# pomonam/LearnablePoolingMethods

Hardware: AMD Instinct MI355X
Metric: clips/sec training step, NetVladV1 K=256 300-frame 1152-d, bs=80, 1/2/4/8 GPU (higher is better)
Workload: dtype f32

## Files before the change

include/lpm_hip.h:

```cpp
#ifndef LPM_HIP_H
#define LPM_HIP_H

#include <stddef.h>
#include <stdint.h>

#ifdef __cplusplus
extern "C" {
#endif

#define LPM_VERSION 100

typedef void* lpm_stream_t;

enum {
    LPM_OK = 0,
    LPM_ERR_BADARG = -1,
    LPM_ERR_UNSUPPORTED_SHAPE = -2,
    LPM_ERR_WORKSPACE = -3,
    LPM_ERR_LAUNCH = -4
};

enum {
    LPM_VLAD_SOFTMAX = 1,
    LPM_VLAD_RESIDUAL = 2,
// ... 352 lines not shown
                          const float* corr_b, float* dk, int64_t ldd, const float* moments, lpm_stream_t stream);
int lpm_mha_bwd_x3_bn_image_fmt(const float* q, const float* k, const float* v, int64_t ld, const float* o, const float* dout, int64_t ldo,
                                const float* lse, int B, int L, int h, int d, float scale, const float* key_scale, const float* key_shift,
                                float* dk_plain, const float* corr_a, const float* corr_b, float* dz_partial, void* dqkv_img,
                                const LpmOperandFormat* g_fmt, lpm_stream_t stream);
int lpm_mha_bn_dk_correct_image(const float* q, const float* k, int64_t ld, int B, int L, int h, int d, float scale, const float* corr_a,
                                const float* corr_b, const float* dk_plain, const float* moments, void* dqkv_img,
                                const LpmOperandFormat* g_fmt, lpm_stream_t stream);
int lpm_mha_logit_stats_moments(const float* q, const float* k, int64_t ld, int B, int L, int h, int d, float* partial, float* moments,
                                lpm_stream_t stream);
int lpm_mha_bwd_x3_image(const float* q, const float* k, const float* v, int64_t ld, const void* o, int o_is_image,
                         const float* dout, int64_t ldo, const float* lse, int B, int L, int h, int d, float scale, void* dqkv3,
                         lpm_stream_t stream);
int lpm_mha_fwd_x3_image(const float* q, const float* k, const float* v, int64_t ld, int B, int L, int h, int d, float scale,
                         void* o3, float* lse, lpm_stream_t stream);
size_t lpm_mha_logit_stats_workspace_bytes(int B, int L, int h);
int lpm_mha_logit_stats(const float* q, const float* k, int64_t ld, int B, int L, int h, int d, float* partial,
                        lpm_stream_t stream);
int lpm_bn_small_fwd(const float* x, int M, int C, const float* gamma, const float* beta, float eps, float decay, int act,
                     const float* mul, float* y, float* mean, float* rstd, float* moving_mean, float* moving_var, lpm_stream_t stream);
int lpm_bn_small_bwd(const float* dy, const float* x, int M, int C, const float* gamma, const float* beta, const float* mean,
                     const float* rstd, int act, const float* mul, float* dx, float* dgamma, float* dbeta, float* dmul,
                     lpm_stream_t stream);
int lpm_mha_bn_corrections(const float* partial, int nblk, int L, const float* mean, const float* var, const float* kscale, float eps,
                           int64_t n, float* dgamma, float* dbeta, float* corr_a, float* corr_b, lpm_stream_t stream);

int lpm_moe_ce_nblk(int B, int V);
int lpm_moe_ce_fwd(const float* gate_act, const float* expert_act, const float* labels, int B, int V, int num_mixtures, float eps,
                   float* predictions, float* loss, float* loss_partial, lpm_stream_t stream);
int lpm_moe_ce_bwd(const float* gate_act, const float* expert_act, const float* labels, const float* dloss,
                   const float* dpredictions, int B, int V, int num_mixtures, float eps, float* dgate_act, float* dexpert_act,
                   lpm_stream_t stream);

#define LPM_ARENA_ALIGN 4096
size_t lpm_clip_adam_scratch_bytes(int64_t total, int ntensors);
int lpm_multi_tensor_clip_adam(float* param, const float* grad, float* m, float* v, const int64_t* offsets,
                               int ntensors, int64_t total, float clip_norm, float lr, float beta1, float beta2,
                               float eps, int64_t step, float* scratch, lpm_stream_t stream);
int lpm_multi_tensor_clip_adam_l2(float* param, const float* grad, float* m, float* v, const int64_t* offsets, const float* l2coef,
                                  int ntensors, int64_t total, float clip_norm, float lr, float beta1, float beta2, float eps,
                                  int64_t step, float* scratch, lpm_stream_t stream);

size_t lpm_factored_clip_adam_scratch_bytes(int N1, int N2);
int lpm_factored_clip_adam(const void* xt, const void* dyt, int R, int N1, int N2, float* param, float* m, float* v,
                           float clip_norm, float lr, float beta1, float beta2, float eps, int64_t step, float* scratch,
                           size_t scratch_bytes, lpm_stream_t stream);
int lpm_factored_clip_adam_q(const void* xt, const void* dyt, const float* x, int64_t ldx, const void* gdt, int R, int N1, int N2,
                             float* param, float* m, float* v, float clip_norm, float lr, float beta1, float beta2, float eps,
                             int64_t step, float* scratch, size_t scratch_bytes, lpm_stream_t stream);
int lpm_factored_clip_adam_copy(const void* xt, const void* dyt, const float* x, int64_t ldx, const void* gdt, int R, int N1, int N2,
                                float* param, float* m, float* v, void* param_bf16, float clip_norm, float lr, float beta1, float beta2,
                                float eps, int64_t step, float* scratch, size_t scratch_bytes, lpm_stream_t stream);
int lpm_factored_fold_supported(int R, int N1, int N2);
int lpm_factored_clip_adam_copy_dx(const void* xt, const void* dyt, const float* x, int64_t ldx, const void* gdt, int R, int N1, int N2,
                                   float* param, float* m, float* v, void* param_bf16, const void* dy_bf16, float* dx, int64_t ld_dx,
                                   float clip_norm, float lr, float beta1, float beta2, float eps, int64_t step, float* scratch,
                                   size_t scratch_bytes, lpm_stream_t stream);

int lpm_dropout_keep_mask(void* mask, int64_t n, float keep_prob, uint64_t seed, lpm_stream_t stream);

int lpm_topk_rows(const float* p, int B, int V, int k, int32_t* index, float* value, lpm_stream_t stream);

int lpm_eval_rows(const float* p, const unsigned char* labels, int B, int V, int k, unsigned char* hit1, int32_t* num_labels,
                  int32_t* hits_at_n, double* loss_row, int32_t* top_index, float* top_value, unsigned char* top_label, lpm_stream_t stream);

#ifdef __cplusplus
// ... 4 lines not shown
```

learnablepoolingmethods_amd/_capi.py:

```python
from __future__ import annotations

import ctypes as C
import os
from typing import Optional

import torch

_HERE = os.path.dirname(os.path.abspath(__file__))
LIB_PATH = os.path.join(_HERE, "_lib", "liblpm_hip.so")

LPM_VLAD_SOFTMAX = 1
LPM_VLAD_RESIDUAL = 2
LPM_VLAD_OUT_KMAJOR = 4
LPM_VLAD_NRM_RAW = 8
LPM_VLAD_OUT_BF16 = 16
LPM_VLAD_TILES_BF16 = 32
LPM_VLAD_NRM_BF16 = 64
LPM_VLAD_RAW_KMAJOR = 128
LPM_VLAD_DEBUG_FALLBACK = 256
LPM_VLAD_WIDE_ALL = 512
LPM_VLAD_WIDE_NONE = 1024

_f = C.c_void_p
_i = C.c_int
# ... 113 lines not shown
    "lpm_bn_rows_fwd": (_i, [_f, _i, _i, _f, _f, _fl, _fl, _i, _f, _f, _f, _f, _f, _f, _s, _f]),
    "lpm_bn_bwd_workspace_bytes": (_s, [_i, _i]),
    "lpm_bn_bwd": (_i, [_f, _f, _f, _f, _f, _fl, _i, _i, _f, _f, _f, _f, _s, _f]),
    "lpm_bn_bwd_x16": (_i, [_f, _f, _f, _f, _f, _fl, _i, _i, _f, _f, _f, _f, _s, _f]),
    "lpm_split_rows": (_i, [_f, _l, _l, _i, _f, _i, _i, _f, _f]),
    "lpm_split_weight": (_i, [_f, _i, _i, _f, _f, _f]),
    "lpm_split_rows_relu_bwd_workspace_bytes": (_s, [_l, _i]),
    "lpm_bias_act_fwd": (_i, [_f, _f, _i, _l, _i, _f]),
    "lpm_bias_act_bwd_workspace_bytes": (_s, [_l, _i]),
    "lpm_bias_act_bwd": (_i, [_f, _f, _i, _l, _i, _f, _f, _f, _s, _f]),
    "lpm_split_rows_relu_bwd": (_i, [_f, _l, _i, _f, _f, _f, _f, _s, _f]),
    "lpm_layer_norm_workspace_bytes": (_s, [_i, _i]),
    "lpm_layer_norm_fwd": (_i, [_f, _f, _f, _f, _i, _i, _i, _fl, _f, _f, _f, _f, _s, _f]),
    "lpm_layer_norm_bwd": (_i, [_f, _f, _f, _f, _i, _i, _i, _f, _f, _f, _f, _s, _f]),
    "lpm_layer_norm_act_fwd": (_i, [_f, _f, _i, _f, _f, _f, _i, _i, _i, _fl, _f, _l, _f, _f, _f, _s, _f]),
    "lpm_layer_norm_pair_fwd": (_i, [_f, _f, _i, _f, _f, _f, _f, _f, _i, _i, _i, _fl, _f, _l, _f, _f, _f, _f, _f, _s, _f]),
    "lpm_layer_norm_act_bwd": (_i, [_f, _l, _f, _f, _f, _f, _f, _i, _i, _i, _i, _f, _f, _f, _f, _f, _f, _f, _f, _s, _f]),
    "lpm_layer_norm_act_mask_image_fwd": (_i, [_f, _f, _i, _f, _fl, _f, _f, _f, _i, _i, _i, _fl, _f, _l, _f, _f, _f, _f, _s, _f]),
    "lpm_layer_norm_act_mask_bwd": (_i, [_f, _l, _f, _f, _f, _f, _f, _i, _f, _fl, _i, _i, _i, _f, _f, _f, _f, _f, _f, _f, _f, _s, _f]),
    "lpm_layer_norm_act_mask_bwd_fmt": (_i, [_f, _l, _f, _f, _f, _f, _f, _i, _f, _fl, _i, _i, _i, _f, _f, _f, _f, _f, _f, _f, _f, _s, _f, _f]),
    "lpm_mha_fwd": (_i, [_f, _f, _f, _l, _i, _i, _i, _i, _fl, _f, _f, _f, _l, _f, _f]),
    "lpm_mha_fwd_x3": (_i, [_f, _f, _f, _l, _i, _i, _i, _i, _fl, _f, _f, _f, _l, _f, _f]),
    "lpm_mha_bwd": (_i, [_f, _f, _f, _l, _f, _f, _l, _f, _i, _i, _i, _i, _fl, _f, _f, _f, _f, _f, _l, _f, _f, _f, _f]),
    "lpm_mha_bn_dk_correct": (_i, [_f, _f, _l, _i, _i, _i, _i, _fl, _f, _f, _f, _l, _f, _f]),
    "lpm_mha_logit_stats_moments": (_i, [_f, _f, _l, _i, _i, _i, _i, _f, _f, _f]),
    "lpm_mha_bwd_x3": (_i, [_f, _f, _f, _l, _f, _f, _l, _f, _i, _i, _i, _i, _fl, _f, _f, _f, _f, _f, _l, _f, _f, _f, _f]),
    "lpm_mha_bwd_x3_image": (_i, [_f, _f, _f, _l, _f, _i, _f, _l, _f, _i, _i, _i, _i, _fl, _f, _f]),
    "lpm_mha_fwd_x3_image": (_i, [_f, _f, _f, _l, _i, _i, _i, _i, _fl, _f, _f, _f]),
    "lpm_mha_logit_stats_workspace_bytes": (_s, [_i, _i, _i]),
    "lpm_mha_logit_stats": (_i, [_f, _f, _l, _i, _i, _i, _i, _f, _f]),
    "lpm_moe_ce_nblk": (_i, [_i, _i]),
    "lpm_moe_ce_fwd": (_i, [_f, _f, _f, _i, _i, _i, _fl, _f, _f, _f, _f]),
    "lpm_moe_ce_bwd": (_i, [_f, _f, _f, _f, _f, _i, _i, _i, _fl, _f, _f, _f]),
    "lpm_clip_adam_scratch_bytes": (_s, [_l, _i]),
    "lpm_factored_clip_adam_scratch_bytes": (_s, [_i, _i]),
    "lpm_factored_clip_adam_q": (_i, [_f, _f, _f, _l, _f, _i, _i, _i, _f, _f, _f, _fl, _fl, _fl, _fl, _fl, _l, _f, _s, _f]),
    "lpm_factored_clip_adam_copy": (_i, [_f, _f, _f, _l, _f, _i, _i, _i, _f, _f, _f, _f, _fl, _fl, _fl, _fl, _fl, _l, _f, _s, _f]),
    "lpm_factored_clip_adam_copy_dx": (_i, [_f, _f, _f, _l, _f, _i, _i, _i, _f, _f, _f, _f, _f, _f, _l, _fl, _fl, _fl, _fl, _fl, _l, _f, _s, _f]),
    "lpm_factored_fold_supported": (_i, [_i, _i, _i]),
    "lpm_factored_clip_adam": (_i, [_f, _f, _i, _i, _i, _f, _f, _f, _fl, _fl, _fl, _fl, _fl, _l, _f, _s, _f]),
    "lpm_multi_tensor_clip_adam": (_i, [_f, _f, _f, _f, _f, _i, _l, _fl, _fl, _fl, _fl, _fl, _l, _f, _f]),
    "lpm_dropout_keep_mask": (_i, [_f, _l, _fl, C.c_uint64, _f]),
    "lpm_topk_rows": (_i, [_f, _i, _i, _i, _f, _f, _f]),
    "lpm_eval_rows": (_i, [_f, _f, _i, _i, _i, _f, _f, _f, _f, _f, _f, _f, _f]),
    "lpm_multi_tensor_clip_adam_l2": (_i, [_f, _f, _f, _f, _f, _f, _i, _l, _fl, _fl, _fl, _fl, _fl, _l, _f, _f]),
    "lpm_weight_pack": (_i, [_f, _i, _f]),
    "lpm_sum_splits": (_i, [_f, _i, _i, _i, _f, _f, _f, _i, _f]),
    "lpm_split_rows_fmt": (_i, [_f, _l, _l, _i, _f, _i, _i, _f, _f, _f, _f]),
    "lpm_split_rows_relu_bwd_fmt": (_i, [_f, _l, _i, _fl, _f, _i, _f, _f, _f, _s, _f, _f]),
    "lpm_split_weight_fmt": (_i, [_f, _i, _i, _f, _f, _i, _f]),
    "lpm_split_weight_tiles_fmt": (_i, [_f, _i, _i, _i, _f, _i, _f]),
    "lpm_split_rows_tiles_fmt": (_i, [_f, _l, _i, _i, _i, _f, _f, _f]),
    "lpm_image_row_tiles_fmt": (_i, [_f, _i, _i, _i, _f, _i, _f]),
    "lpm_dense_tiles_act_image_fwd_fmt": (_i, [_f, _i, _f, _f, _i, _i, _i, _fl, _f, _f, _f]),
    "lpm_dense_tiles_relu_bwd_image_fmt": (_i, [_f, _i, _f, _f, _i, _i, _i, _i, _fl, _f, _f, _f, _s, _f, _f]),
    "lpm_layer_norm_act_image_fwd_fmt": (_i, [_f, _f, _i, _f, _f, _f, _f, _i, _i, _i, _fl, _f, _l, _f, _f, _f, _f, _s, _f, _f]),
    "lpm_layer_norm_act_mask_image_fwd_fmt": (_i, [_f, _f, _i, _f, _fl, _f, _f, _f, _i, _i, _i, _fl, _f, _l, _f, _f, _f, _f, _s, _f, _f]),
    "lpm_layer_norm_act_bwd_fmt": (_i, [_f, _l, _f, _f, _f, _f, _f, _i, _i, _i, _i, _f, _f, _f, _f, _f, _f, _f, _f, _s, _f, _f]),
    "lpm_mha_fwd_x3_image_fmt": (_i, [_f, _f, _f, _l, _i, _i, _i, _i, _fl, _f, _f, _f, _f]),
    "lpm_mha_bwd_x3_image_fmt": (_i, [_f, _f, _f, _l, _f, _f, _f, _l, _f, _i, _i, _i, _i, _fl, _f, _f, _f]),
    "lpm_sum_splits_scaled": (_i, [_f, _i, _i, _i, _i, _fl, _f, _f, _f, _i, _f]),
    "lpm_mha_bwd_x3_bn_image_fmt": (_i, [_f, _f, _f, _l, _f, _f, _l, _f, _i, _i, _i, _i, _fl, _f, _f, _f, _f, _f, _f, _f, _f, _f]),
    "lpm_mha_bn_dk_correct_image": (_i, [_f, _f, _l, _i, _i, _i, _i, _fl, _f, _f, _f, _f, _f, _f, _f]),
    "lpm_bn_rows_act_image_fwd_fmt": (_i, [_f, _f, _i, _i, _i, _f, _f, _fl, _fl, _i, _f, _f, _f, _f, _f, _f, _s, _f, _f]),
    "lpm_bn_act_bwd_image_fmt": (_i, [_f, _f, _f, _i, _f, _f, _f, _fl, _i, _i, _f, _f, _f, _f, _f, _s, _f, _f]),
}
# ... 70 lines not shown
```

learnablepoolingmethods_amd/csrc/moe_head.hip:

```cpp
#include "lpm_common.h"

namespace lpm {

constexpr int MOE_MAX_MIX = 8;

__device__ __forceinline__ void moe_mix(const float* __restrict__ ga, const float* __restrict__ ea, int m, float* g, float* e, float* ne,
                                        float& p, float& q) {
    float mx = ga[0];
    for (int i = 1; i <= m; ++i) mx = fmaxf(mx, ga[i]);
    float s = 0.f;
    for (int i = 0; i <= m; ++i) {
        g[i] = __expf(ga[i] - mx);
        s += g[i];
    }
    const float inv = 1.f / s;
    p = 0.f;
    for (int i = 0; i <= m; ++i) g[i] *= inv;
    q = g[m];
    for (int i = 0; i < m; ++i) {
        const float a = ea[i], t = __expf(-fabsf(a)), r = 1.f / (1.f + t);
        const float big = r, small = t * r;
        e[i] = a >= 0.f ? big : small;
        ne[i] = a >= 0.f ? small : big;
        p = fmaf(g[i], e[i], p);
// ... 26 lines not shown

__global__ __launch_bounds__(256) void moe_ce_loss_reduce_kernel(const float* __restrict__ partial, int nblk, float inv_batch,
                                                                 float* __restrict__ loss) {
    __shared__ double sh[256];
    double s = 0.0;
    for (int i = threadIdx.x; i < nblk; i += 256) s += (double)partial[i];
    sh[threadIdx.x] = s;
    __syncthreads();
    for (int o = 128; o > 0; o >>= 1) {
        if (threadIdx.x < o) sh[threadIdx.x] += sh[threadIdx.x + o];
        __syncthreads();
    }
    if (threadIdx.x == 0) loss[0] = (float)(sh[0] * (double)inv_batch);
}

__global__ __launch_bounds__(256) void moe_ce_bwd_kernel(const float* __restrict__ gate_act, const float* __restrict__ expert_act,
                                                         const float* __restrict__ labels, const float* __restrict__ dloss,
                                                         const float* __restrict__ dpred, int64_t n, int m, float eps,
                                                         float inv_batch, float* __restrict__ dgate, float* __restrict__ dexpert) {
    const int64_t i = (int64_t)blockIdx.x * 256 + threadIdx.x;
    if (i >= n) return;
    float g[MOE_MAX_MIX + 1], e[MOE_MAX_MIX], ne[MOE_MAX_MIX], p, q;
    moe_mix(gate_act + i * (m + 1), expert_act + i * m, m, g, e, ne, p, q);
    float dp = dpred ? dpred[i] : 0.f;
    if (labels && dloss) {
        const float y = labels[i];
        dp += dloss[0] * inv_batch * -(y / (p + eps) - (1.f - y) / (q + eps));
    }
    for (int j = 0; j < m; ++j) {
        dexpert[i * m + j] = dp * g[j] * e[j] * ne[j];
        dgate[i * (m + 1) + j] = dp * g[j] * (q - ne[j]);
    }
    dgate[i * (m + 1) + m] = dp * g[m] * (0.f - p);
}

}

extern "C" int lpm_moe_ce_nblk(int B, int V) { return (int)(((int64_t)B * V + 255) / 256); }

extern "C" int lpm_moe_ce_fwd(const float* gate_act, const float* expert_act, const float* labels, int B, int V, int num_mixtures,
                              float eps, float* predictions, float* loss, float* loss_partial, lpm_stream_t stream) {
    using namespace lpm;
    LPM_REQUIRE(gate_act && expert_act && predictions, LPM_ERR_BADARG, "lpm_moe_ce_fwd: null pointer");
    LPM_REQUIRE((labels == nullptr) == (loss == nullptr) && (loss == nullptr) == (loss_partial == nullptr), LPM_ERR_BADARG,
                "lpm_moe_ce_fwd: labels, loss and loss_partial go together");
    LPM_REQUIRE(B > 0 && V > 0 && num_mixtures >= 1 && num_mixtures <= MOE_MAX_MIX, LPM_ERR_UNSUPPORTED_SHAPE,
                "lpm_moe_ce_fwd: need 1 <= num_mixtures <= %d (got %d)", MOE_MAX_MIX, num_mixtures);
    const int64_t n = (int64_t)B * V;
    const int nblk = lpm_moe_ce_nblk(B, V);
    hipStream_t s = (hipStream_t)stream;
    hipLaunchKernelGGL(moe_ce_fwd_kernel, dim3(nblk), dim3(256), 0, s, gate_act, expert_act, labels, n, num_mixtures, eps, predictions,
                       loss_partial);
    if (loss) hipLaunchKernelGGL(moe_ce_loss_reduce_kernel, dim3(1), dim3(256), 0, s, loss_partial, nblk, 1.f / (float)B, loss);
    return check_launch("lpm_moe_ce_fwd");
}

extern "C" int lpm_moe_ce_bwd(const float* gate_act, const float* expert_act, const float* labels, const float* dloss,
                              const float* dpredictions, int B, int V, int num_mixtures, float eps, float* dgate_act,
                              float* dexpert_act, lpm_stream_t stream) {
    using namespace lpm;
    LPM_REQUIRE(gate_act && expert_act && dgate_act && dexpert_act, LPM_ERR_BADARG, "lpm_moe_ce_bwd: null pointer");
    LPM_REQUIRE((labels == nullptr) == (dloss == nullptr), LPM_ERR_BADARG, "lpm_moe_ce_bwd: labels and dloss go together");
    LPM_REQUIRE(B > 0 && V > 0 && num_mixtures >= 1 && num_mixtures <= MOE_MAX_MIX, LPM_ERR_UNSUPPORTED_SHAPE,
                "lpm_moe_ce_bwd: need 1 <= num_mixtures <= %d (got %d)", MOE_MAX_MIX, num_mixtures);
    const int64_t n = (int64_t)B * V;
    hipLaunchKernelGGL(moe_ce_bwd_kernel, dim3(lpm_moe_ce_nblk(B, V)), dim3(256), 0, (hipStream_t)stream, gate_act, expert_act, labels, dloss,
                       dpredictions, n, num_mixtures, eps, 1.f / (float)B, dgate_act, dexpert_act);
    return check_launch("lpm_moe_ce_bwd");
}
```

learnablepoolingmethods_amd/ops.py:

```python
from __future__ import annotations

import ctypes as C
import os
import weakref
from typing import NamedTuple, Optional

import torch

from . import _capi
from ._capi import LPM_VLAD_NRM_RAW, LPM_VLAD_OUT_KMAJOR, LPM_VLAD_RESIDUAL, LPM_VLAD_SOFTMAX, LpmError, ptr, stream_ptr

BN_EPS = 1e-3
BN_DECAY = 0.999

VLAD_PRECISION = os.environ.get("LPM_VLAD_PRECISION", "bf16x3")
VLAD_TILES3 = os.environ.get("LPM_VLAD_TILES3", "1") != "0"
VLAD_FUSED = os.environ.get("LPM_VLAD_FUSED", "0") == "1"
PROJ_STREAM = os.environ.get("LPM_PROJ_STREAM", "1") != "0"
PROJ_DX_STREAM_MIN_N = int(os.environ.get("LPM_PROJ_DX_STREAM_MIN_N", "512"))
BN_ACT_FUSED = os.environ.get("LPM_BN_ACT_FUSED", "1") != "0"
BIAS_ACT_FUSED = os.environ.get("LPM_BIAS_ACT_FUSED", "1") != "0"
FACTORED_NORM_QUADFORM = os.environ.get("LPM_FACTORED_NORM_QUADFORM", "1") != "0"
VLAD_SOFTMAX_FUSED = os.environ.get("LPM_VLAD_SOFTMAX_FUSED", "0") == "1"
FRAME_ROW_TILES = os.environ.get("LPM_FRAME_ROW_TILES", "0") == "1"
VLAD_FUSED_DEBUG_FALLBACK = False

VLAD_KMAJOR_SCALED = os.environ.get("LPM_VLAD_KMAJOR_SCALED", "0") == "1"
VLAD_CLIP = os.environ.get("LPM_VLAD_CLIP", "1") != "0"
VLAD_CLIP16 = os.environ.get("LPM_VLAD_CLIP16", "1") != "0"
FFN_TILES = os.environ.get("LPM_FFN_TILES", "1") != "0"
DIRECT_WGRAD = True
FFN_MOD_FUSED = os.environ.get("LPM_FFN_MOD_FUSED", "1") != "0"
ASSIGN_PRECISION = os.environ.get("LPM_ASSIGN_PRECISION", "bf16x3")

MHA_PRECISION = os.environ.get("LPM_MHA_PRECISION", "bf16x3")
MHA_BN_PRECISION = os.environ.get("LPM_MHA_BN_PRECISION", "mixed")
MHA_BN_MIXED = os.environ.get("LPM_MHA_BN_MIXED", "auto,bf16x3,bf16x3")
MHA_BN_X3_MIN_KEYS = int(os.environ.get("LPM_MHA_BN_X3_MIN_KEYS", "128"))

_XT_CACHE = {}
MHA_BN_MOMENTS = os.environ.get("LPM_MHA_BN_MOMENTS", "1") != "0"
MHA_BN_ONEPASS = os.environ.get("LPM_MHA_BN_ONEPASS", "1") != "0"
LN_IMAGE = os.environ.get("LPM_LN_IMAGE", "1") != "0"
SPLIT_VECTOR = True
V2_SPLIT_COLUMNS = True
DEBUG_TAP = None

KERNEL_TIMELINE = None


class _timed:
    def __init__(self, name, dims):
        self.name, self.dims = name, dims

    def __enter__(self):
        if KERNEL_TIMELINE is not None:
            self.t0 = torch.cuda.Event(enable_timing=True)
            self.t1 = torch.cuda.Event(enable_timing=True)
            self.t0.record()
        return self

    def __exit__(self, *exc):
        if KERNEL_TIMELINE is not None:
            self.t1.record()
            KERNEL_TIMELINE.append((self.name, self.dims, self.t0, self.t1))
        return False


def _f32(t: torch.Tensor, what: str) -> torch.Tensor:
    if t.dtype != torch.float32:
        raise LpmError(f"{what}: expected float32, got {t.dtype}")
    return t


# ... 2888 lines not shown
        if labels is not None:
            labels = labels.to(device=gate_act.device, dtype=torch.float32).contiguous()
            loss = _empty((), gate_act)
            part = _empty((lib._lpm_moe_ce_nblk(B, V),), gate_act)
        lib.check(lib._lpm_moe_ce_fwd(ptr(gate_act), ptr(expert_act), ptr(labels), B, V, num_mixtures, eps, ptr(pred), ptr(loss),
                                      ptr(part), stream_ptr()), "lpm_moe_ce_fwd")
        ctx.dims = (B, V, num_mixtures, eps)
        ctx.save_for_backward(gate_act, expert_act, labels)
        ctx.set_materialize_grads(False)
        if labels is None:
            ctx.mark_non_differentiable()
            return pred, None
        return pred, loss

    @staticmethod
    def backward(ctx, dpred, dloss):
        lib = _capi.load()
        B, V, m, eps = ctx.dims
        gate_act, expert_act, labels = ctx.saved_tensors
        dgate, dexpert = torch.empty_like(gate_act), torch.empty_like(expert_act)
        if dloss is None and labels is not None:
            dloss = torch.zeros((), dtype=torch.float32, device=gate_act.device)
        dloss = dloss.contiguous() if dloss is not None else None
        dpred = dpred.contiguous() if dpred is not None else None
        lib.check(lib._lpm_moe_ce_bwd(ptr(gate_act), ptr(expert_act), ptr(labels), ptr(dloss), ptr(dpred), B, V, m, eps, ptr(dgate),
                                      ptr(dexpert), stream_ptr()), "lpm_moe_ce_bwd")
        return dgate, dexpert, None, None, None


def moe_cross_entropy(gate_act, expert_act, labels, num_mixtures, eps=10e-6):
    return _MoeCrossEntropy.apply(gate_act, expert_act, labels, int(num_mixtures), float(eps))


class ComputeCopy:

    def __init__(self, W, also=()):
        self.buf = torch.empty(W.shape, dtype=torch.bfloat16, device=W.device)
        self.also = tuple(also)
        self.version = None
        self.stale = True
        self.refreshes = 0

    def invalidate(self):
        self.stale = True

    def _versions(self, W):
        return (W._version,) + tuple(t._version for t in self.also)

    def tensor(self, W):
        v = self._versions(W)
        if self.stale or self.version != v:
            self.buf.copy_(W.detach())
            self.version, self.stale = v, False
            self.refreshes += 1
        return self.buf

    def current(self, W):
        return None if (self.stale or self.version != self._versions(W)) else self.buf


PROJ_W16 = os.environ.get("LPM_PROJ_W16", "1") != "0"


class FactoredGradient:

    def __init__(self, on_put=None, strict=False):
# ... 149 lines not shown
```

learnablepoolingmethods_amd/video_level_models.py:

```python
from __future__ import annotations

import math

import torch

from . import FLAGS, models
from . import variables as vs


def _linear(x, W, b=None):
    if x.is_cuda and x.dtype == torch.float32 and W.dtype == torch.float32 and x.dim() == 2:
        from . import ops
        return ops.linear_direct(x, W, b)
    return torch.addmm(b, x, W) if b is not None else x.matmul(W)


class MoeModel(models.BaseModel):

    def create_model(self, model_input, vocab_size, is_training=True, num_mixtures=None, l2_penalty=1e-8,
                     labels=None, fused_cross_entropy=False, **unused_params):
        num_mixtures = num_mixtures or FLAGS.moe_num_mixtures
        low_rank_gating = FLAGS.moe_low_rank_gating
        l2_penalty = FLAGS.moe_l2
        gating_probabilities = FLAGS.moe_prob_gating
        gating_input = FLAGS.moe_prob_gating_input
        H = model_input.shape[1]
        dev = model_input.device
        store = vs.default_store()
        if low_rank_gating == -1:
            with vs.variable_scope("gates"):
                wg = vs.get_variable("weights", [H, vocab_size * (num_mixtures + 1)], vs.glorot_uniform_initializer(), device=dev)
            store.add_l2_regularizer(wg, l2_penalty)
            gate_activations = _linear(model_input, wg)
        else:
            with vs.variable_scope("gates1"):
                wg1 = vs.get_variable("weights", [H, low_rank_gating], vs.glorot_uniform_initializer(), device=dev)
            with vs.variable_scope("gates2"):
                wg2 = vs.get_variable("weights", [low_rank_gating, vocab_size * (num_mixtures + 1)], vs.glorot_uniform_initializer(), device=dev)
            store.add_l2_regularizer(wg1, l2_penalty)
            store.add_l2_regularizer(wg2, l2_penalty)
            gate_activations = model_input.matmul(wg1).matmul(wg2)
        with vs.variable_scope("experts"):
            we = vs.get_variable("weights", [H, vocab_size * num_mixtures], vs.glorot_uniform_initializer(), device=dev)
            be = vs.get_variable("biases", [vocab_size * num_mixtures], vs.zeros_initializer(), device=dev)
        store.add_l2_regularizer(we, l2_penalty)
        expert_activations = _linear(model_input, we, be)
        fuse_loss = fused_cross_entropy and not gating_probabilities
        if model_input.is_cuda and num_mixtures <= 8 and (labels is None or fused_cross_entropy):
            from . import ops
            probabilities, loss = ops.moe_cross_entropy(gate_activations, expert_activations,
                                                        labels if fuse_loss else None, num_mixtures)
            if not gating_probabilities:
                return {"predictions": probabilities, "loss": loss} if loss is not None else {"predictions": probabilities}
        else:
            gating_distribution = torch.softmax(gate_activations.reshape(-1, num_mixtures + 1), dim=-1)
            expert_distribution = torch.sigmoid(expert_activations.reshape(-1, num_mixtures))
            probabilities = (gating_distribution[:, :num_mixtures] * expert_distribution).sum(dim=1)
            probabilities = probabilities.reshape(-1, vocab_size)
        if gating_probabilities:
            from . import layers
            rows = vocab_size if gating_input == "prob" else H
            gating_weights = vs.get_variable("gating_prob_weights", [rows, vocab_size],
                                             vs.random_normal_initializer(1 / math.sqrt(vocab_size)), device=dev)
            gates = (probabilities if gating_input == "prob" else model_input).matmul(gating_weights)
            if FLAGS.gating_remove_diag:
                if rows != vocab_size:
                    raise ValueError("gating_remove_diag with moe_prob_gating_input != 'prob': the diagonal of a "
                                     f"[{rows}, {vocab_size}] matrix does not broadcast against the probabilities (as in the reference)")
                gates = gates - torch.diagonal(gating_weights) * probabilities
            gates = layers.batch_norm(gates, is_training, "gating_prob_bn")
            probabilities = probabilities * torch.sigmoid(gates)
        return {"predictions": probabilities}
```

Baseline: 12530.

## Fuse MoE head linear layers with mixture and cross-entropy into one kernel

Adds fused forward and backward HIP kernels that compute the gate and expert linear projections with MFMA, the mixture-of-experts probabilities, and the cross-entropy loss in one pass per column block. The backward also produces weight, bias and input gradients, with input gradients written to per-block slabs and then reduced. This removes separate GEMM launches and the round trips of activations through memory. The cost is extra slab memory and reduction work for dx, plus custom GEMM code that may be slower than a library GEMM for larger shapes. It is only used for full-rank gating with batch size up to 128.

```diff
diff --git a/include/lpm_hip.h b/include/lpm_hip.h
--- a/include/lpm_hip.h
+++ b/include/lpm_hip.h
@@ -408,6 +408,15 @@
                    const float* dpredictions, int B, int V, int num_mixtures, float eps, float* dgate_act, float* dexpert_act,
                    lpm_stream_t stream);
 
+int lpm_moe_head_nblk(int V, int num_mixtures);
+int lpm_moe_head_fwd(const float* x, const float* gate_w, const float* expert_w, const float* expert_b, const void* labels,
+                     int labels_u8, int B, int H, int V, int num_mixtures, float eps, float* gate_act, float* expert_act,
+                     float* predictions, float* loss, float* loss_partial, lpm_stream_t stream);
+int lpm_moe_head_bwd(const float* x, const float* gate_w, const float* expert_w, const float* gate_act, const float* expert_act,
+                     const void* labels, int labels_u8, const float* dloss, const float* dpredictions, int B, int H, int V,
+                     int num_mixtures, float eps, float* dgate_w, float* dexpert_w, float* dexpert_b, float* dx, float* dx_slabs,
+                     lpm_stream_t stream);
+
 #define LPM_ARENA_ALIGN 4096
 size_t lpm_clip_adam_scratch_bytes(int64_t total, int ntensors);
 int lpm_multi_tensor_clip_adam(float* param, const float* grad, float* m, float* v, const int64_t* offsets,
diff --git a/learnablepoolingmethods_amd/_capi.py b/learnablepoolingmethods_amd/_capi.py
--- a/learnablepoolingmethods_amd/_capi.py
+++ b/learnablepoolingmethods_amd/_capi.py
@@ -169,6 +169,9 @@
     "lpm_moe_ce_nblk": (_i, [_i, _i]),
     "lpm_moe_ce_fwd": (_i, [_f, _f, _f, _i, _i, _i, _fl, _f, _f, _f, _f]),
     "lpm_moe_ce_bwd": (_i, [_f, _f, _f, _f, _f, _i, _i, _i, _fl, _f, _f, _f]),
+    "lpm_moe_head_nblk": (_i, [_i, _i]),
+    "lpm_moe_head_fwd": (_i, [_f, _f, _f, _f, _f, _i, _i, _i, _i, _i, _fl, _f, _f, _f, _f, _f, _f]),
+    "lpm_moe_head_bwd": (_i, [_f, _f, _f, _f, _f, _f, _i, _f, _f, _i, _i, _i, _i, _fl, _f, _f, _f, _f, _f, _f]),
     "lpm_clip_adam_scratch_bytes": (_s, [_l, _i]),
     "lpm_factored_clip_adam_scratch_bytes": (_s, [_i, _i]),
     "lpm_factored_clip_adam_q": (_i, [_f, _f, _f, _l, _f, _i, _i, _i, _f, _f, _f, _fl, _fl, _fl, _fl, _fl, _l, _f, _s, _f]),
diff --git a/learnablepoolingmethods_amd/csrc/moe_head.hip b/learnablepoolingmethods_amd/csrc/moe_head.hip
--- a/learnablepoolingmethods_amd/csrc/moe_head.hip
+++ b/learnablepoolingmethods_amd/csrc/moe_head.hip
@@ -82,6 +82,396 @@
         dgate[i * (m + 1) + j] = dp * g[j] * (q - ne[j]);
     }
     dgate[i * (m + 1) + m] = dp * g[m] * (0.f - p);
+}
+
+
+constexpr int MH_NT = 5;
+constexpr int MH_COLS = 16 * MH_NT;
+constexpr int MH_LDT = MH_COLS + 1;
+
+struct HeadCols {
+    int ng, nl;
+    int g0, e0;
+    int gN, eN;
+};
+__device__ __forceinline__ HeadCols head_cols(int blk, int cb, int m, int V) {
+    HeadCols hc;
+    hc.ng = cb * (m + 1);
+    hc.nl = cb * (2 * m + 1);
+    hc.g0 = blk * hc.ng;
+    hc.e0 = blk * cb * m;
+    hc.gN = V * (m + 1);
+    hc.eN = V * m;
+    return hc;
+}
+__device__ __forceinline__ bool head_col(const HeadCols& hc, int c, bool& expert, int& col) {
+    expert = c >= hc.ng;
+    col = expert ? hc.e0 + (c - hc.ng) : hc.g0 + c;
+    return c < hc.nl && col < (expert ? hc.eN : hc.gN);
+}
+__device__ __forceinline__ float head_label(const void* labels, int u8, int64_t i) {
+    return u8 ? (float)((const uint8_t*)labels)[i] : ((const float*)labels)[i];
+}
+
+template <int RT>
+__global__ __launch_bounds__(256) void moe_head_fwd_kernel(const float* __restrict__ x, const float* __restrict__ Wg,
+                                                           const float* __restrict__ We, const float* __restrict__ be,
+                                                           const void* __restrict__ labels, int labels_u8, int B, int H, int V, int m,
+                                                           int cb, float eps, float* __restrict__ gate_act,
+                                                           float* __restrict__ expert_act, float* __restrict__ pred,
+                                                           float* __restrict__ loss_partial) {
+    __shared__ __attribute__((aligned(16))) float T[RT * 16 * MH_LDT];
+    const int blk = xcd_remap(blockIdx.x, gridDim.x);
+    const int lane = threadIdx.x & 63, wave = threadIdx.x >> 6, li = lane & 15, g = lane >> 4;
+    const HeadCols hc = head_cols(blk, cb, m, V);
+
+    const float* wp[MH_NT];
+    int ld[MH_NT];
+#pragma unroll
+    for (int t = 0; t < MH_NT; ++t) {
+        bool ex;
+        int col;
+        const bool ok = head_col(hc, t * 16 + li, ex, col);
+        wp[t] = ok ? (ex ? We : Wg) + col : Wg;
+        ld[t] = (ok && ex) ? hc.eN : hc.gN;
+    }
+    constexpr int NIT = (RT * 16 * 26 + 255) / 256;
+    __shared__ float bias_s[MH_COLS];
+    __shared__ float ys[NIT * 256];
+    if (threadIdx.x < MH_COLS) {
+        bool ex;
+        int col;
+        const bool ok = head_col(hc, threadIdx.x, ex, col);
+        bias_s[threadIdx.x] = (ok && ex) ? be[col] : 0.f;
+    }
+    if (labels) {
+        float yv[NIT];
+        int64_t yi[NIT];
+#pragma unroll
+        for (int it = 0; it < NIT; ++it) {
+            const int i = min((int)threadIdx.x + it * 256, B * cb - 1), r = i / cb;
+            yi[it] = (int64_t)r * V + min(blk * cb + (i - r * cb), V - 1);
+        }
+        if (labels_u8) {
+#pragma unroll
+            for (int it = 0; it < NIT; ++it) yv[it] = (float)((const uint8_t*)labels)[yi[it]];
+        } else {
+#pragma unroll
+            for (int it = 0; it < NIT; ++it) yv[it] = ((const float*)labels)[yi[it]];
+        }
+#pragma unroll
+        for (int it = 0; it < NIT; ++it) ys[threadIdx.x + it * 256] = yv[it];
+    }
+
+    f32x4 acc[RT][MH_NT];
+#pragma unroll
+    for (int rt = 0; rt < RT; ++rt)
+#pragma unroll
+        for (int t = 0; t < MH_NT; ++t) acc[rt][t] = f32x4{0.f, 0.f, 0.f, 0.f};
+
+    const int nch = H >> 4, ch0 = wave * nch / 4, ch1 = (wave + 1) * nch / 4;
+    auto load = [&](int ch, float (&w)[4][MH_NT], f32x4 (&xv)[RT]) {
+        const int k = ch * 16 + 4 * g;
+#pragma unroll
+        for (int s = 0; s < 4; ++s)
+#pragma unroll
+            for (int t = 0; t < MH_NT; ++t) w[s][t] = wp[t][(int64_t)(k + s) * ld[t]];
+#pragma unroll
+        for (int rt = 0; rt < RT; ++rt) xv[rt] = *(const f32x4*)(x + (int64_t)min(rt * 16 + li, B - 1) * H + k);
+    };
+    float w0[4][MH_NT], w1[4][MH_NT], w2[4][MH_NT];
+    f32x4 x0[RT], x1[RT], x2[RT];
+    auto step = [&](int next, float (&wc)[4][MH_NT], f32x4 (&xc)[RT], float (&wn)[4][MH_NT], f32x4 (&xn)[RT]) {
+        load(min(next, ch1 - 1), wn, xn);
+        __builtin_amdgcn_sched_barrier(0);
+#pragma unroll
+        for (int s = 0; s < 4; ++s)
+#pragma unroll
+            for (int rt = 0; rt < RT; ++rt)
+#pragma unroll
+                for (int t = 0; t < MH_NT; ++t) acc[rt][t] = mfma16(xc[rt][s], wc[s][t], acc[rt][t]);
+        __builtin_amdgcn_sched_barrier(0);
+    };
+    if (ch0 < ch1) {
+        load(ch0, w0, x0);
+        load(min(ch0 + 1, ch1 - 1), w1, x1);
+        for (int ch = ch0; ch < ch1; ch += 3) {
+            step(ch + 2, w0, x0, w2, x2);
+            if (ch + 1 >= ch1) break;
+            step(ch + 3, w1, x1, w0, x0);
+            if (ch + 2 >= ch1) break;
+            step(ch + 4, w2, x2, w1, x1);
+        }
+    }
+
+    f32x4* stage = (f32x4*)T;
+    for (int src = 3; src >= 1; --src) {
+        if (wave == src) {
+#pragma unroll
+            for (int rt = 0; rt < RT; ++rt)
+#pragma unroll
+                for (int t = 0; t < MH_NT; ++t) stage[(rt * MH_NT + t) * 64 + lane] = acc[rt][t];
+        }
+        __syncthreads();
+        if (wave == src - 1) {
+#pragma unroll
+            for (int rt = 0; rt < RT; ++rt)
+#pragma unroll
+                for (int t = 0; t < MH_NT; ++t) acc[rt][t] += stage[(rt * MH_NT + t) * 64 + lane];
+        }
+    }
+    __syncthreads();
+    if (wave == 0) {
+#pragma unroll
+        for (int rt = 0; rt < RT; ++rt)
+#pragma unroll
+            for (int t = 0; t < MH_NT; ++t)
+#pragma unroll
+                for (int j = 0; j < 4; ++j) T[(rt * 16 + 4 * g + j) * MH_LDT + t * 16 + li] = acc[rt][t][j];
+    }
+    __syncthreads();
+
+    for (int i = threadIdx.x; i < B * MH_COLS; i += 256) {
+        const int r = i / MH_COLS, c = i - r * MH_COLS;
+        bool ex;
+        int col;
+        if (!head_col(hc, c, ex, col)) continue;
+        const float v = T[r * MH_LDT + c] + bias_s[c];
+        if (ex) {
+            T[r * MH_LDT + c] = v;
+            if (expert_act) expert_act[(int64_t)r * hc.eN + col] = v;
+        } else if (gate_act) {
+            gate_act[(int64_t)r * hc.gN + col] = v;
+        }
+    }
+    __syncthreads();
+    float l = 0.f;
+    for (int i = threadIdx.x; i < B * cb; i += 256) {
+        const int r = i / cb, cl = i - r * cb, cls = blk * cb + cl;
+        if (cls >= V) continue;
+        float gg[MOE_MAX_MIX + 1], e[MOE_MAX_MIX], ne[MOE_MAX_MIX], p, q;
+        moe_mix(T + r * MH_LDT + cl * (m + 1), T + r * MH_LDT + hc.ng + cl * m, m, gg, e, ne, p, q);
+        pred[(int64_t)r * V + cls] = p;
+        if (labels) {
+            const float y = ys[i];
+            l += -(y * __logf(p + eps) + (1.f - y) * __logf(q + eps));
+        }
+    }
+    if (loss_partial) {
+        l = wave_sum(l);
+        __shared__ float w[4];
+        if (lane == 0) w[wave] = l;
+        __syncthreads();
+        if (threadIdx.x == 0) loss_partial[blk] = (w[0] + w[1]) + (w[2] + w[3]);
+    }
+}
+
+template <int RT>
+__global__ __launch_bounds__(256) void moe_head_bwd_kernel(const float* __restrict__ x, const float* __restrict__ Wg,
+                                                           const float* __restrict__ We, const float* __restrict__ gate_act,
+                                                           const float* __restrict__ expert_act, const void* __restrict__ labels,
+                                                           int labels_u8, const float* __restrict__ dloss,
+                                                           const float* __restrict__ dpred, int B, int H, int V, int m, int cb, float eps,
+                                                           float* __restrict__ dWg, float* __restrict__ dWe, float* __restrict__ dbe,
+                                                           float* __restrict__ dx_slabs) {
+    __shared__ __attribute__((aligned(16))) float T[RT * 16 * MH_LDT];
+    const int blk = xcd_remap(blockIdx.x, gridDim.x);
+    const int lane = threadIdx.x & 63, wave = threadIdx.x >> 6, li = lane & 15, g = lane >> 4;
+    const HeadCols hc = head_cols(blk, cb, m, V);
+
+    constexpr int NCP = RT * 16 * MH_COLS / 256, NIT = (RT * 16 * 26 + 255) / 256;
+    const int nitem = B * cb;
+    float yv[NIT], dpv[NIT];
+    {
+        float v[NCP];
+#pragma unroll
+        for (int it = 0; it < NCP; ++it) {
+            const int i = threadIdx.x + it * 256, r = i / MH_COLS, c = i - r * MH_COLS;
+            bool ex;
+            int col;
+            const bool ok = head_col(hc, c, ex, col) && r < B;
+            const float* src = !ok ? gate_act : ex ? expert_act + (int64_t)r * hc.eN + col : gate_act + (int64_t)r * hc.gN + col;
+            v[it] = *src;
+        }
+        int64_t yi[NIT];
+#pragma unroll
+        for (int it = 0; it < NIT; ++it) {
+            const int i = min((int)threadIdx.x + it * 256, nitem - 1), r = i / cb;
+            yi[it] = (int64_t)r * V + min(blk * cb + (i - r * cb), V - 1);
+            yv[it] = 0.f;
+            dpv[it] = 0.f;
+        }
+        if (labels && dloss) {
+            if (labels_u8) {
+#pragma unroll
+                for (int it = 0; it < NIT; ++it) yv[it] = (float)((const uint8_t*)labels)[yi[it]];
+            } else {
+#pragma unroll
+                for (int it = 0; it < NIT; ++it) yv[it] = ((const float*)labels)[yi[it]];
+            }
+        }
+        if (dpred) {
+#pragma unroll
+            for (int it = 0; it < NIT; ++it) dpv[it] = dpred[yi[it]];
+        }
+#pragma unroll
+        for (int it = 0; it < NCP; ++it) {
+            const int i = threadIdx.x + it * 256, r = i / MH_COLS, c = i - r * MH_COLS;
+            bool ex;
+            int col;
+            const bool ok = head_col(hc, c, ex, col) && r < B;
+            T[r * MH_LDT + c] = ok ? v[it] : 0.f;
+        }
+    }
+    __syncthreads();
+    const float inv_batch = 1.f / (float)B, dl = (labels && dloss) ? dloss[0] * inv_batch : 0.f;
+#pragma unroll
+    for (int it = 0; it < NIT; ++it) {
+        const int i = threadIdx.x + it * 256, r = i / cb, cl = i - r * cb, cls = blk * cb + cl;
+        if (i >= nitem || cls >= V) continue;
+        float* tg = T + r * MH_LDT + cl * (m + 1);
+        float* te = T + r * MH_LDT + hc.ng + cl * m;
+        float gg[MOE_MAX_MIX + 1], e[MOE_MAX_MIX], ne[MOE_MAX_MIX], p, q;
+        moe_mix(tg, te, m, gg, e, ne, p, q);
+        float dp = dpv[it];
+        if (labels && dloss) {
+            const float y = yv[it];
+            dp += dl * -(y / (p + eps) - (1.f - y) / (q + eps));
+        }
+        for (int j = 0; j < m; ++j) {
+            te[j] = dp * gg[j] * e[j] * ne[j];
+            tg[j] = dp * gg[j] * (q - ne[j]);
+        }
+        tg[m] = dp * gg[m] * (0.f - p);
+    }
+    __syncthreads();
+
+    if (dbe && threadIdx.x < MH_COLS) {
+        bool ex;
+        int col;
+        if (head_col(hc, threadIdx.x, ex, col) && ex) {
+            float s = 0.f;
+#pragma unroll 8
+            for (int r = 0; r < B; ++r) s += T[r * MH_LDT + threadIdx.x];
+            dbe[col] = s;
+        }
+    }
+
+    const int nht = H >> 4, ht0 = wave * nht / 4, ht1 = (wave + 1) * nht / 4;
+    constexpr int KS = 4 * RT;
+    if ((dWg || dWe) && ht0 < ht1) {
+        float df[KS][MH_NT];
+#pragma unroll
+        for (int ks = 0; ks < KS; ++ks)
+#pragma unroll
+            for (int t = 0; t < MH_NT; ++t) df[ks][t] = T[(4 * ks + g) * MH_LDT + t * 16 + li];
+        float* op[MH_NT];
+        int old[MH_NT];
+#pragma unroll
+        for (int t = 0; t < MH_NT; ++t) {
+            bool ex;
+            int col;
+            const bool ok = head_col(hc, t * 16 + li, ex, col);
+            float* base = ex ? dWe : dWg;
+            op[t] = (ok && base) ? base + col : nullptr;
+            old[t] = ex ? hc.eN : hc.gN;
+        }
+        float xa[KS];
+        auto loadx = [&](int ht, float (&a)[KS]) {
+#pragma unroll
+            for (int ks = 0; ks < KS; ++ks) a[ks] = x[(int64_t)min(4 * ks + g, B - 1) * H + ht * 16 + li];
+        };
+        loadx(ht0, xa);
+        for (int ht = ht0; ht < ht1; ++ht) {
+            float xn[KS];
+            loadx(min(ht + 1, ht1 - 1), xn);
+            __builtin_amdgcn_sched_barrier(0);
+            f32x4 acc[MH_NT];
+#pragma unroll
+            for (int t = 0; t < MH_NT; ++t) acc[t] = f32x4{0.f, 0.f, 0.f, 0.f};
+#pragma unroll
+            for (int ks = 0; ks < KS; ++ks)
+#pragma unroll
+                for (int t = 0; t < MH_NT; ++t) acc[t] = mfma16(xa[ks], df[ks][t], acc[t]);
+#pragma unroll
+            for (int t = 0; t < MH_NT; ++t)
+                if (op[t]) {
+#pragma unroll
+                    for (int j = 0; j < 4; ++j) op[t][(int64_t)(ht * 16 + 4 * g + j) * old[t]] = acc[t][j];
+                }
+#pragma unroll
+            for (int ks = 0; ks < KS; ++ks) xa[ks] = xn[ks];
+        }
+    }
+
+    if (dx_slabs && ht0 < ht1) {
+        constexpr int KC = MH_COLS / 4;
+        float* slab = dx_slabs + (int64_t)blk * B * H;
+        const float* wq[KC];
+        int wld[KC];
+#pragma unroll
+        for (int ks = 0; ks < KC; ++ks) {
+            bool ex;
+            int col;
+            const bool ok = head_col(hc, 4 * ks + g, ex, col);
+            wq[ks] = ok ? (ex ? We : Wg) + col : Wg;
+            wld[ks] = (ok && ex) ? hc.eN : hc.gN;
+        }
+        auto loadw = [&](int ht, float (&w)[KC]) {
+#pragma unroll
+            for (int ks = 0; ks < KC; ++ks) w[ks] = wq[ks][(int64_t)(ht * 16 + li) * wld[ks]];
+        };
+        float wa0[KC], wa1[KC], wa2[KC];
+        auto step = [&](int ht, float (&wc)[KC], float (&wn)[KC]) {
+            loadw(min(ht + 2, ht1 - 1), wn);
+            __builtin_amdgcn_sched_barrier(0);
+            f32x4 acc[RT];
+#pragma unroll
+            for (int rt = 0; rt < RT; ++rt) acc[rt] = f32x4{0.f, 0.f, 0.f, 0.f};
+#pragma unroll
+            for (int ks = 0; ks < KC; ++ks)
+#pragma unroll
+                for (int rt = 0; rt < RT; ++rt) acc[rt] = mfma16(T[(rt * 16 + li) * MH_LDT + 4 * ks + g], wc[ks], acc[rt]);
+#pragma unroll
+            for (int rt = 0; rt < RT; ++rt)
+#pragma unroll
+                for (int j = 0; j < 4; ++j) {
+                    const int b = rt * 16 + 4 * g + j;
+                    if (b < B) slab[(int64_t)b * H + ht * 16 + li] = acc[rt][j];
+                }
+            __builtin_amdgcn_sched_barrier(0);
+        };
+        loadw(ht0, wa0);
+        loadw(min(ht0 + 1, ht1 - 1), wa1);
+        for (int ht = ht0; ht < ht1; ht += 3) {
+            step(ht, wa0, wa2);
+            if (ht + 1 >= ht1) break;
+            step(ht + 1, wa1, wa0);
+            if (ht + 2 >= ht1) break;
+            step(ht + 2, wa2, wa1);
+        }
+    }
+}
+
+__global__ __launch_bounds__(256) void moe_head_dx_reduce_kernel(const f32x4* __restrict__ slabs, int nblk, int64_t n4,
+                                                                 f32x4* __restrict__ dx) {
+    __shared__ f32x4 sh[3][64];
+    const int lane = threadIdx.x & 63, wave = threadIdx.x >> 6;
+    const int64_t e = (int64_t)blockIdx.x * 64 + lane;
+    f32x4 s = f32x4{0.f, 0.f, 0.f, 0.f};
+    if (e < n4) {
+        const int b0 = wave * nblk / 4, b1 = (wave + 1) * nblk / 4;
+        for (int b = b0; b < b1; b += 8) {
+            f32x4 v[8];
+#pragma unroll
+            for (int u = 0; u < 8; ++u) v[u] = (b + u < b1) ? slabs[(int64_t)(b + u) * n4 + e] : f32x4{0.f, 0.f, 0.f, 0.f};
+#pragma unroll
+            for (int u = 0; u < 8; ++u) s += v[u];
+        }
+    }
+    if (wave > 0) sh[wave - 1][lane] = s;
+    __syncthreads();
+    if (wave == 0 && e < n4) dx[e] = ((s + sh[0][lane]) + sh[1][lane]) + sh[2][lane];
 }
 
 }
@@ -118,3 +508,70 @@
                        dpredictions, n, num_mixtures, eps, 1.f / (float)B, dgate_act, dexpert_act);
     return check_launch("lpm_moe_ce_bwd");
 }
+
+static int moe_head_cb(int num_mixtures) { return lpm::MH_COLS / (2 * num_mixtures + 1); }
+
+extern "C" int lpm_moe_head_nblk(int V, int num_mixtures) {
+    if (V <= 0 || num_mixtures < 1 || num_mixtures > lpm::MOE_MAX_MIX) return 0;
+    const int cb = moe_head_cb(num_mixtures);
+    return (V + cb - 1) / cb;
+}
+
+static int moe_head_check(const char* what, int B, int H, int V, int m) {
+    using namespace lpm;
+    LPM_REQUIRE(B >= 1 && B <= 128, LPM_ERR_UNSUPPORTED_SHAPE, "%s: need 1 <= B <= 128 (got %d)", what, B);
+    LPM_REQUIRE(H >= 16 && H % 16 == 0, LPM_ERR_UNSUPPORTED_SHAPE, "%s: need H a multiple of 16 (got %d)", what, H);
+    LPM_REQUIRE(V > 0 && m >= 1 && m <= MOE_MAX_MIX, LPM_ERR_UNSUPPORTED_SHAPE, "%s: need 1 <= num_mixtures <= %d (got %d)", what,
+                MOE_MAX_MIX, m);
+    LPM_REQUIRE((int64_t)V * (m + 1) * H < ((int64_t)1 << 31), LPM_ERR_UNSUPPORTED_SHAPE, "%s: weight matrix too large", what);
+    return LPM_OK;
+}
+
+extern "C" int lpm_moe_head_fwd(const float* x, const float* gate_w, const float* expert_w, const float* expert_b, const void* labels,
+                                int labels_u8, int B, int H, int V, int num_mixtures, float eps, float* gate_act, float* expert_act,
+                                float* predictions, float* loss, float* loss_partial, lpm_stream_t stream) {
+    using namespace lpm;
+    LPM_REQUIRE(x && gate_w && expert_w && expert_b && predictions, LPM_ERR_BADARG, "lpm_moe_head_fwd: null pointer");
+    LPM_REQUIRE((labels == nullptr) == (loss == nullptr) && (loss == nullptr) == (loss_partial == nullptr), LPM_ERR_BADARG,
+                "lpm_moe_head_fwd: labels, loss and loss_partial go together");
+    LPM_REQUIRE((gate_act == nullptr) == (expert_act == nullptr), LPM_ERR_BADARG,
+                "lpm_moe_head_fwd: gate_act and expert_act go together");
+    LPM_REQUIRE(((uintptr_t)x & 15) == 0, LPM_ERR_BADARG, "lpm_moe_head_fwd: x must be 16-byte aligned");
+    if (int rc = moe_head_check("lpm_moe_head_fwd", B, H, V, num_mixtures)) return rc;
+    const int nblk = lpm_moe_head_nblk(V, num_mixtures), cb = moe_head_cb(num_mixtures);
+    hipStream_t s = (hipStream_t)stream;
+    if (B <= 80)
+        hipLaunchKernelGGL(moe_head_fwd_kernel<5>, dim3(nblk), dim3(256), 0, s, x, gate_w, expert_w, expert_b, labels, labels_u8, B, H, V,
+                           num_mixtures, cb, eps, gate_act, expert_act, predictions, loss_partial);
+    else
+        hipLaunchKernelGGL(moe_head_fwd_kernel<8>, dim3(nblk), dim3(256), 0, s, x, gate_w, expert_w, expert_b, labels, labels_u8, B, H, V,
+                           num_mixtures, cb, eps, gate_act, expert_act, predictions, loss_partial);
+    if (loss) hipLaunchKernelGGL(moe_ce_loss_reduce_kernel, dim3(1), dim3(256), 0, s, loss_partial, nblk, 1.f / (float)B, loss);
+    return check_launch("lpm_moe_head_fwd");
+}
+
+extern "C" int lpm_moe_head_bwd(const float* x, const float* gate_w, const float* expert_w, const float* gate_act,
+                                const float* expert_act, const void* labels, int labels_u8, const float* dloss,
+                                const float* dpredictions, int B, int H, int V, int num_mixtures, float eps, float* dgate_w,
+                                float* dexpert_w, float* dexpert_b, float* dx, float* dx_slabs, lpm_stream_t stream) {
+    using namespace lpm;
+    LPM_REQUIRE(x && gate_w && expert_w && gate_act && expert_act, LPM_ERR_BADARG, "lpm_moe_head_bwd: null pointer");
+    LPM_REQUIRE((labels == nullptr) == (dloss == nullptr), LPM_ERR_BADARG, "lpm_moe_head_bwd: labels and dloss go together");
+    LPM_REQUIRE((dx == nullptr) == (dx_slabs == nullptr), LPM_ERR_BADARG, "lpm_moe_head_bwd: dx and dx_slabs go together");
+    LPM_REQUIRE((((uintptr_t)dx | (uintptr_t)dx_slabs) & 15) == 0, LPM_ERR_BADARG, "lpm_moe_head_bwd: dx and dx_slabs must be 16-byte aligned");
+    if (int rc = moe_head_check("lpm_moe_head_bwd", B, H, V, num_mixtures)) return rc;
+    const int nblk = lpm_moe_head_nblk(V, num_mixtures), cb = moe_head_cb(num_mixtures);
+    hipStream_t s = (hipStream_t)stream;
+    if (B <= 80)
+        hipLaunchKernelGGL(moe_head_bwd_kernel<5>, dim3(nblk), dim3(256), 0, s, x, gate_w, expert_w, gate_act, expert_act, labels, labels_u8,
+                           dloss, dpredictions, B, H, V, num_mixtures, cb, eps, dgate_w, dexpert_w, dexpert_b, dx_slabs);
+    else
+        hipLaunchKernelGGL(moe_head_bwd_kernel<8>, dim3(nblk), dim3(256), 0, s, x, gate_w, expert_w, gate_act, expert_act, labels, labels_u8,
+                           dloss, dpredictions, B, H, V, num_mixtures, cb, eps, dgate_w, dexpert_w, dexpert_b, dx_slabs);
+    if (dx) {
+        const int64_t n4 = (int64_t)B * H / 4;
+        hipLaunchKernelGGL(moe_head_dx_reduce_kernel, dim3((unsigned)((n4 + 63) / 64)), dim3(256), 0, s, (const f32x4*)dx_slabs, nblk, n4,
+                           (f32x4*)dx);
+    }
+    return check_launch("lpm_moe_head_bwd");
+}
diff --git a/learnablepoolingmethods_amd/ops.py b/learnablepoolingmethods_amd/ops.py
--- a/learnablepoolingmethods_amd/ops.py
+++ b/learnablepoolingmethods_amd/ops.py
@@ -40,6 +40,7 @@
 
 _XT_CACHE = {}
 MHA_BN_MOMENTS = os.environ.get("LPM_MHA_BN_MOMENTS", "1") != "0"
+MOE_HEAD = os.environ.get("LPM_MOE_HEAD", "1") != "0"
 MHA_BN_ONEPASS = os.environ.get("LPM_MHA_BN_ONEPASS", "1") != "0"
 LN_IMAGE = os.environ.get("LPM_LN_IMAGE", "1") != "0"
 SPLIT_VECTOR = True
@@ -2994,6 +2995,99 @@
     return _MoeCrossEntropy.apply(gate_act, expert_act, labels, int(num_mixtures), float(eps))
 
 
+MOE_HEAD_MAX_BATCH = 128
+
+
+def moe_head_shapes_ok(B, H, wg_shape, we_shape, be_shape, num_mixtures, labels_shape=None):
+    m = int(num_mixtures)
+    if not (1 <= m <= 8 and 1 <= B <= MOE_HEAD_MAX_BATCH and H >= 16 and H % 16 == 0):
+        return False
+    if len(wg_shape) != 2 or len(we_shape) != 2 or len(be_shape) != 1 or wg_shape[0] != H or we_shape[0] != H:
+        return False
+    V = wg_shape[1] // (m + 1)
+    if V < 1 or wg_shape[1] != V * (m + 1) or we_shape[1] != V * m or be_shape[0] != V * m or wg_shape[1] * H >= 2 ** 31:
+        return False
+    return labels_shape is None or tuple(labels_shape) == (B, V)
+
+
+def moe_head_ok(x, Wg, We, be, labels, num_mixtures):
+    if not (MOE_HEAD and x.is_cuda and x.dim() == 2 and all(t.is_cuda and t.dtype == torch.float32 for t in (x, Wg, We, be))):
+        return False
+    if not (Wg.is_contiguous() and We.is_contiguous() and be.is_contiguous()):
+        return False
+    if labels is not None and not (labels.is_cuda and labels.dtype in (torch.bool, torch.uint8, torch.float32)):
+        return False
+    return moe_head_shapes_ok(x.shape[0], x.shape[1], Wg.shape, We.shape, be.shape, num_mixtures,
+                              None if labels is None else labels.shape)
+
+
+class _MoeHead(torch.autograd.Function):
+
+    @staticmethod
+    def forward(ctx, x, Wg, We, be, labels, m, eps):
+        lib = _capi.load()
+        B, H = x.shape
+        V = Wg.shape[1] // (m + 1)
+        if not x.is_contiguous() or x.data_ptr() % 16:
+            x = x.contiguous() if not x.is_contiguous() else x.clone()
+        if labels is not None and not labels.is_contiguous():
+            labels = labels.contiguous()
+        keep = any(ctx.needs_input_grad[:4])
+        pred = _empty((B, V), x)
+        gate_act = _empty((B, V * (m + 1)), x) if keep else None
+        expert_act = _empty((B, V * m), x) if keep else None
+        loss = part = None
+        if labels is not None:
+            loss = _empty((), x)
+            part = _empty((lib._lpm_moe_head_nblk(V, m),), x)
+        u8 = int(labels is not None and labels.dtype != torch.float32)
+        lib.check(lib._lpm_moe_head_fwd(ptr(x), ptr(Wg), ptr(We), ptr(be), ptr(labels), u8, B, H, V, m, eps, ptr(gate_act),
+                                        ptr(expert_act), ptr(pred), ptr(loss), ptr(part), stream_ptr()), "lpm_moe_head_fwd")
+        ctx.dims = (B, H, V, m, eps, u8)
+        ctx.wrefs = (Wg, We)
+        if keep:
+            ctx.save_for_backward(x, Wg, We, gate_act, expert_act, labels)
+        ctx.set_materialize_grads(False)
+        if labels is None:
+            return pred, None
+        return pred, loss
+
+    @staticmethod
+    def backward(ctx, dpred, dloss):
+        lib = _capi.load()
+        B, H, V, m, eps, u8 = ctx.dims
+        x, Wg, We, gate_act, expert_act, labels = ctx.saved_tensors
+        if dloss is None and labels is not None:
+            dloss = torch.zeros((), dtype=torch.float32, device=x.device)
+        dloss = dloss.contiguous() if dloss is not None else None
+        dpred = dpred.contiguous() if dpred is not None else None
+        grads, direct = [None, None], [False, False]
+        for k, W in enumerate(ctx.wrefs):
+            if ctx.needs_input_grad[1 + k]:
+                slot = _grad_slot(W)
+                direct[k] = slot is not None and slot.is_contiguous() and slot.shape == W.shape
+                grads[k] = slot if direct[k] else torch.empty_like(W, memory_format=torch.contiguous_format)
+        dWg, dWe = grads
+        dbe = _empty((V * m,), x) if ctx.needs_input_grad[3] else None
+        dx = slabs = None
+        if ctx.needs_input_grad[0]:
+            dx = _empty((B, H), x)
+            slabs = _empty((lib._lpm_moe_head_nblk(V, m), B, H), x)
+        lib.check(lib._lpm_moe_head_bwd(ptr(x), ptr(Wg), ptr(We), ptr(gate_act), ptr(expert_act), ptr(labels), u8, ptr(dloss), ptr(dpred),
+                                        B, H, V, m, eps, ptr(dWg), ptr(dWe), ptr(dbe), ptr(dx), ptr(slabs), stream_ptr()),
+                  "lpm_moe_head_bwd")
+        for k, W in enumerate(ctx.wrefs):
+            if direct[k]:
+                _grad_done(W)
+        return dx, None if direct[0] else dWg, None if direct[1] else dWe, dbe, None, None, None
+
+
+def moe_head(x, Wg, We, be, labels, num_mixtures, eps=10e-6):
+    if not moe_head_ok(x, Wg, We, be, labels, num_mixtures):
+        raise LpmError("moe_head: unsupported arguments (see ops.moe_head_ok); use linear_direct + moe_cross_entropy")
+    return _MoeHead.apply(x, Wg, We, be, labels, int(num_mixtures), float(eps))
+
+
 class ComputeCopy:
 
     def __init__(self, W, also=()):
diff --git a/learnablepoolingmethods_amd/video_level_models.py b/learnablepoolingmethods_amd/video_level_models.py
--- a/learnablepoolingmethods_amd/video_level_models.py
+++ b/learnablepoolingmethods_amd/video_level_models.py
@@ -31,7 +31,6 @@
             with vs.variable_scope("gates"):
                 wg = vs.get_variable("weights", [H, vocab_size * (num_mixtures + 1)], vs.glorot_uniform_initializer(), device=dev)
             store.add_l2_regularizer(wg, l2_penalty)
-            gate_activations = _linear(model_input, wg)
         else:
             with vs.variable_scope("gates1"):
                 wg1 = vs.get_variable("weights", [H, low_rank_gating], vs.glorot_uniform_initializer(), device=dev)
@@ -44,19 +43,28 @@
             we = vs.get_variable("weights", [H, vocab_size * num_mixtures], vs.glorot_uniform_initializer(), device=dev)
             be = vs.get_variable("biases", [vocab_size * num_mixtures], vs.zeros_initializer(), device=dev)
         store.add_l2_regularizer(we, l2_penalty)
-        expert_activations = _linear(model_input, we, be)
         fuse_loss = fused_cross_entropy and not gating_probabilities
-        if model_input.is_cuda and num_mixtures <= 8 and (labels is None or fused_cross_entropy):
+        on_gpu = model_input.is_cuda and num_mixtures <= 8 and (labels is None or fused_cross_entropy)
+        head_labels = labels if fuse_loss else None
+        probabilities = loss = None
+        if on_gpu:
             from . import ops
-            probabilities, loss = ops.moe_cross_entropy(gate_activations, expert_activations,
-                                                        labels if fuse_loss else None, num_mixtures)
-            if not gating_probabilities:
-                return {"predictions": probabilities, "loss": loss} if loss is not None else {"predictions": probabilities}
-        else:
-            gating_distribution = torch.softmax(gate_activations.reshape(-1, num_mixtures + 1), dim=-1)
-            expert_distribution = torch.sigmoid(expert_activations.reshape(-1, num_mixtures))
-            probabilities = (gating_distribution[:, :num_mixtures] * expert_distribution).sum(dim=1)
-            probabilities = probabilities.reshape(-1, vocab_size)
+            if low_rank_gating == -1 and ops.moe_head_ok(model_input, wg, we, be, head_labels, num_mixtures):
+                probabilities, loss = ops.moe_head(model_input, wg, we, be, head_labels, num_mixtures)
+        if probabilities is None:
+            if low_rank_gating == -1:
+                gate_activations = _linear(model_input, wg)
+            expert_activations = _linear(model_input, we, be)
+            if on_gpu:
+                probabilities, loss = ops.moe_cross_entropy(gate_activations, expert_activations, head_labels,
+                                                            num_mixtures)
+            else:
+                gating_distribution = torch.softmax(gate_activations.reshape(-1, num_mixtures + 1), dim=-1)
+                expert_distribution = torch.sigmoid(expert_activations.reshape(-1, num_mixtures))
+                probabilities = (gating_distribution[:, :num_mixtures] * expert_distribution).sum(dim=1)
+                probabilities = probabilities.reshape(-1, vocab_size)
+        if on_gpu and not gating_probabilities:
+            return {"predictions": probabilities, "loss": loss} if loss is not None else {"predictions": probabilities}
         if gating_probabilities:
             from . import layers
             rows = vocab_size if gating_input == "prob" else H
```

After: 12620, median of 6. No clear change (+0.7%).
